# earth-system-radiation/rte-ecckd

Measured on AMD Instinct MI355X. Metric: Mcol*lay*gpt/s LW gas_optics+rte_lw, higher is better.
Workload: dtype f64

## Files before the change

rte-ecckd_amd/csrc/capi.cpp:

```cpp
#include <hip/hip_runtime.h>

#include <atomic>
#include <cmath>
#include <cstdint>
#include <cstdlib>
#include <cstring>
#include <map>
#include <mutex>
#include <string>
#include <vector>

#include "../../include/ecckd_hip.h"
#include "kernels.hpp"
#include "model.hpp"

namespace {

thread_local std::string g_err;

int fail(const std::string &msg) {
  g_err = msg;
  return 1;
}
}
// ... 205 lines not shown

struct Bump {
  char *base;
  size_t es;
  size_t off = 0;
  Bump(void *b, bool f32) : base(static_cast<char *>(b)), es(esz(f32)) {}
  double *take(size_t nelem) {
    double *r = reinterpret_cast<double *>(base + off);
    off += align256(nelem * es);
    return r;
  }
};

struct GasDesc {
  int ngas;
  const char *names;
  const double *const *vmr;
  const long long *cs, *ls;
  const double *scalar;
};

size_t vmr_extent(const GasDesc &gd, int j, int ncol, int nlay) {
  if (!gd.vmr || !gd.vmr[j]) return 0;
  const long long cs = gd.cs ? gd.cs[j] : 0, ls = gd.ls ? gd.ls[j] : 0;
  return (size_t)(1 + (long long)(ncol - 1) * cs + (long long)(nlay - 1) * ls);
}

struct PlanckSide {
  const double *tlev, *tsfc;
  double *lay_source, *lev_inc, *lev_dec, *sfc_source;
};

ecckd::PlanckArgs planck_args(const ecckd_model *m, int ncol, int nlay, const double *tlay, const PlanckSide &pl) {
  ecckd::PlanckArgs p{};
  p.ncol = ncol; p.nlay = nlay; p.ng = m->ng; p.ntp = m->ntp;
  p.planck = m->dbuf + m->off_planck;
  p.t0 = m->temperature_planck[0];
  p.dt = m->temperature_planck[1] - m->temperature_planck[0];
  p.tlay = tlay; p.tlev = pl.tlev; p.tsfc = pl.tsfc;
  p.lay_source = pl.lay_source; p.lev_source_inc = pl.lev_inc; p.lev_source_dec = pl.lev_dec;
  p.sfc_source = pl.sfc_source;
  return p;
}

int planck_sources_dev(const ecckd_model *m, int ncol, int nlay, const double *tlay, const PlanckSide &pl,
                       hipStream_t stream) {
  ecckd::PlanckArgs p = planck_args(m, ncol, nlay, tlay, pl);
  ProfScope prof("planck", stream);
  if (g_arith.load() == 0) HIPCHK(ecckd::launch_planck_pair(p, 0, stream));
  else HIPCHK(ecckd::launch_planck(p, stream));
  return 0;
}

int gas_optical_depth_dev(const ecckd_model *m, bool f32, PlanRecord *plan, int ncol, int nlay, const double *plev,
                          const double *tlay, const GasDesc &gd, double *tau, bool sw, double *ssa,
                          double *g, const PlanckSide *pl, bool *planck_done, hipStream_t stream) {
  using namespace ecckd;
  if (planck_done) *planck_done = false;
  std::vector<SeqGas> seq;
  bool first_calc = true;
  for (int j = 0; j < gd.ngas; ++j) {
    const std::string name = trim_name(gd.names + (size_t)j * ECCKD_NAME_LEN);
    size_t i = 0;
    for (; i < m->gas.size(); ++i)
      if (m->gas[i].name == name) break;
    if (i >= m->gas.size()) continue;
    const ecckd_model::Gas &t = m->gas[i];
    if (t.composite_only && !first_calc) continue;
    SeqGas e{};
    e.coef = table(m, t.dev_off, f32);
    e.vmr = gd.vmr ? gd.vmr[j] : nullptr;
    e.cs = gd.cs ? gd.cs[j] : 0;
    e.ls = gd.ls ? gd.ls[j] : 0;
    e.scalar = gd.scalar ? gd.scalar[j] : 0.;
    if (plan) {
      const bool sc = plan->is_scalar && plan->is_scalar[j];
      e.vmr = sc ? nullptr : reinterpret_cast<const double *>(sizeof(double));
      e.scalar = 1.;
    }
    e.ref = t.ref;
    e.code = t.code;
    e.nv = t.nv;
    e.clamp = t.has_negative ? 1 : 0;
    if (t.code == ECCKD_LOOK_UP_TABLE) {
      e.mf0 = t.mole_fraction[0];
      e.log_mf0 = std::log(t.mole_fraction[0]);
      e.d_log_vmr = std::log(t.mole_fraction[1] / t.mole_fraction[0]);
    }
    seq.push_back(e);
    if (t.composite_only) first_calc = false;
  }

  const bool fast = g_arith.load() == 0;
  size_t pos = 0;
  bool first_pass = true;
  do {
    FusedArgs fa{};
    TauArgs &a = fa.tau;
    a.ncol = ncol; a.nlay = nlay; a.ng = m->ng; a.np = m->np; a.nt = m->nt;
    a.plev = plev; a.tlay = tlay;
    a.temperature = table(m, m->off_temperature, f32);
    a.zero = table(m, m->off_zero, f32);
    a.lp0 = m->log_pressure[0];
    a.dlp = m->log_pressure[1] - m->log_pressure[0];
    a.dt = m->temperature[m->np] - m->temperature[0];
    a.gw = gw(f32);
    a.lut = -1;
    a.merge_slot = -1;
    a.nmerge = 0;
    a.nbil = 0;
    a.nseq = 0;
    while (pos < seq.size()) {
      SeqGas e = seq[pos];
      if (a.nseq >= kTauPassGases) break;
      if (e.code == ECCKD_LOOK_UP_TABLE) {
        if (a.lut >= 0) break;
        a.lut = a.nseq;
      } else {
        e.slot = a.nbil;
        a.bil_seq[a.nbil++] = a.nseq;
      }
      a.seq[a.nseq++] = e;
      ++pos;
    }
    a.accumulate = first_pass ? 0 : 1;
    a.tau = tau;
    const bool last = pos >= seq.size();
    if (sw && last) {
      a.rayleigh = table(m, m->off_rayleigh, f32);
      a.ssa = ssa;
      a.g = g;
    }
    if (fast) {
      fa.mode = (sw && last) ? 2 : 0;
      if (g_opt.gas_merge_scalars.load() && !f32) merge_scalar_gases(a, f32);
      const int nv_lut = a.lut >= 0 ? a.seq[a.lut].nv : 0;
      int pass_clamp = 0;
      for (int k = 0; k < a.nseq; ++k) pass_clamp |= a.seq[k].clamp;
      if (pl && first_pass && !sw &&
          fused_planck_rows(a.ng, a.np, a.nt, a.nbil, nv_lut, m->ntp, pass_clamp, f32) > 0) {
        fa.mode = 1;
        fa.ntp = m->ntp;
        fa.planck = table(m, m->off_planck, f32);
        fa.pt0 = m->temperature_planck[0];
        fa.pdt = m->temperature_planck[1] - m->temperature_planck[0];
        fa.tlev = pl->tlev; fa.tsfc = pl->tsfc;
        fa.lay_source = pl->lay_source; fa.lev_source_inc = pl->lev_inc;
        fa.lev_source_dec = pl->lev_dec; fa.sfc_source = pl->sfc_source;
        if (planck_done) *planck_done = true;
      }
      fa.f32 = f32;
      ScratchLease flag_lease;
      fa.slab32 = (!f32 && !plan && m->f32_exact && fa.mode == 1) ? g_opt.gas_slab_f32.load() : 0;
      if (fa.slab32 == 2) fa.choose_buf = static_cast<int *>(stream_scratch_optional(m->device, stream, 256, flag_lease, g_flag_pool));
      if (f32 && ((fa.mode != 1 && fa.mode != 2) || !last || !first_pass))
        return fail("ecckd: single precision is implemented for one-pass gas optics (fused longwave, shortwave); this "
                    "model / gas list needs the multi-pass or unfused path");
      if (plan) {
        FusedPlan fp;
        HIPCHK(prepare_gas_fused(fa, fp));
        if (plan->npass == 0) { plan->first_fused = 1; plan->planck_fused = fa.mode == 1; plan->first = fp; }
        ++plan->npass;
      } else {
        ProfScope prof(fa.mode == 1 ? (f32 ? "gas_lw_fused_f32" : "gas_lw_fused") : "tau", stream);
        HIPCHK(launch_gas_fused(fa, stream));
      }
    } else {
      if (f32) return fail("ecckd: single precision needs the fast arithmetic mode (ecckd_set_arithmetic(0))");
      if (plan) {
        ++plan->npass;
      } else {
        ProfScope prof("tau", stream);
        HIPCHK(launch_tau(a, stream));
      }
    }
    first_pass = false;
  } while (pos < seq.size());
  return 0;
}

int check_model(const ecckd_model *m) {
  if (!m) return fail("ecckd: null model");
  if (!m->finalized) return fail("ecckd: model is not finalized");
  if (m->device < 0) return fail("ecckd: host-only model (device -1): no GPU, no compute (there is no CPU fallback)");
  return 0;
}

int check_dims(int ncol, int nlay) {
  if (ncol < 0 || nlay < 1) return fail("ecckd: bad ncol/nlay");
  return 0;
}
int check_gas_optics_dims(int ncol, int nlay) {
  if (check_dims(ncol, nlay)) return 1;
  if (((size_t)ncol * (size_t)nlay + (size_t)ncol) * sizeof(double) >= (size_t)0xFFFFFFF0u)
    return fail("ecckd: ncol*(nlay+1) too large for one call (limit 2^29 elements): split the column range");
  return 0;
}

struct StagedGases {
  std::vector<const double *> ptr;
  GasDesc gd;
};
size_t staged_gas_bytes(const GasDesc &gd, int ncol, int nlay, bool f32) {
  size_t b = 0;
  for (int j = 0; j < gd.ngas; ++j) b += align256(vmr_extent(gd, j, ncol, nlay) * esz(f32));
  return b;
}
int stage_gases(const GasDesc &gd, int ncol, int nlay, Bump &bump, hipStream_t s, StagedGases &out) {
  out.ptr.assign(gd.ngas, nullptr);
  for (int j = 0; j < gd.ngas; ++j) {
    const size_t n = vmr_extent(gd, j, ncol, nlay);
    if (!n) continue;
    double *d = bump.take(n);
    HIPCHK(hipMemcpyAsync(d, gd.vmr[j], n * bump.es, hipMemcpyHostToDevice, s));
    out.ptr[j] = d;
  }
  out.gd = gd;
  out.gd.vmr = out.ptr.data();
  return 0;
}

int h2d(double *d, const double *h, size_t n, bool f32, hipStream_t s) {
  HIPCHK(hipMemcpyAsync(d, h, n * esz(f32), hipMemcpyHostToDevice, s));
  return 0;
}
int d2h(double *h, const double *d, size_t n, bool f32, hipStream_t s) {
  HIPCHK(hipMemcpyAsync(h, d, n * esz(f32), hipMemcpyDeviceToHost, s));
  return 0;
}

int grow_arena(ecckd_model *m, size_t need) {
  if (need <= m->arena_bytes) return 0;
  HIPCHK(hipStreamSynchronize(m->host_stream));
  if (m->arena) { HIPCHK(hipFree(m->arena)); m->arena = nullptr; m->arena_bytes = 0; }
  HIPCHK(hipMalloc(&m->arena, need));
  m->arena_bytes = need;
  return 0;
}

template <class T> void sum_planes_host(const T *planes, int nplanes, size_t n, T *out) {
  for (size_t i = 0; i < n; ++i) {
    T acc = 0;
    for (int b = 0; b < nplanes; ++b) acc += planes[(size_t)b * n + i];
    out[i] = acc;
  }
}

int sum_planes(const double *planes, int nplanes, size_t n, double *out, bool f32, int memspace, void *stream) {
  if (memspace == ECCKD_DEVICE) {
    HIPCHK(ecckd::launch_sum_planes(planes, nplanes, n, out, f32, static_cast<hipStream_t>(stream)));
    return 0;
  }
  if (f32)
    sum_planes_host(reinterpret_cast<const float *>(planes), nplanes, n, reinterpret_cast<float *>(out));
  else
    sum_planes_host(planes, nplanes, n, out);
  return 0;
}
template <class T> T *el(T *p, size_t n, bool f32) { return reinterpret_cast<T *>(reinterpret_cast<uintptr_t>(p) + n * esz(f32)); }

int fill_band_map(int ngpt, int nband, const int *band2gpt, unsigned char *gpt2band) {
  if (ngpt < 1 || ngpt > 256) return fail("ecckd: ngpt must be in 1..256");
  if (nband < 1 || nband > 255 || !band2gpt) return fail("ecckd: bad band description");
  std::memset(gpt2band, 0, 256);
  std::vector<int> seen(ngpt, 0);
  for (int b = 0; b < nband; ++b) {
    const int lo = band2gpt[2 * b], hi = band2gpt[2 * b + 1];
    if (lo < 1 || hi > ngpt || lo > hi) return fail("ecckd: band2gpt out of range");
    for (int gpt = lo; gpt <= hi; ++gpt) { gpt2band[gpt - 1] = (unsigned char)b; seen[gpt - 1] = 1; }
  }
  for (int i = 0; i < ngpt; ++i)
    if (!seen[i]) return fail("ecckd: band2gpt does not cover every g-point");
  return 0;
}

}

extern "C" {

const char *ecckd_last_error(void) { return g_err.c_str(); }

const char *ecckd_build_info(void) {
  return "rte-ecckd hot path for MI355X: hipcc --offload-arch=gfx950 -O3 -ffp-contract=off, fp64";
}


int ecckd_device_malloc(int device, size_t bytes, void **ptr) {
  if (!ptr) return fail("ecckd_device_malloc: null output");
  *ptr = nullptr;
  int ndev = 0;
  if (hipGetDeviceCount(&ndev) != hipSuccess || ndev < 1)
    return fail("ecckd: no HIP device available (this library has no CPU fallback)");
  if (device < 0 || device >= ndev) return fail("ecckd_device_malloc: bad device ordinal");
  HIPCHK(hipSetDevice(device));
  if (bytes == 0) return 0;
  HIPCHK(hipMalloc(ptr, bytes));
  return 0;
}

int ecckd_device_free(int device, void *ptr) {
  if (!ptr) return 0;
  HIPCHK(hipSetDevice(device));
  HIPCHK(hipFree(ptr));
  return 0;
}

int ecckd_device_memcpy(int device, void *dst, const void *src, size_t bytes, int to_device) {
// ... 1310 lines not shown
```

rte-ecckd_amd/csrc/kernels.hpp:

```cpp
#pragma once
#include <hip/hip_runtime.h>

namespace ecckd {

constexpr int kMaxSeq = 16;
constexpr int kTauPassGases = 10;
constexpr int kLdsBudget = 160 * 1024;

struct SeqGas {
  const double *coef;
  const double *vmr;
  long long cs, ls;
  double scalar;
  double ref;
  double mf0;
  double log_mf0;
  double d_log_vmr;
  int code;
  int nv;
  int slot;
  int clamp;
};

struct TauArgs {
  int ncol, nlay, ng, np, nt;
  const double *plev, *tlay;
  const double *temperature;
  const double *zero;
  double lp0, dlp, dt, gw;
  int nseq;
  SeqGas seq[kMaxSeq];
  int nbil;
  int bil_seq[kMaxSeq];
  int lut;
  int merge_slot;
  int nmerge;
  int merge_seq[kMaxSeq];
  double merge_mult[kMaxSeq];
  int accumulate;
  double *tau;
  const double *rayleigh;
  double *ssa, *g;
  int R;
  int col_chunks;
  int seg;
};

struct UDiv { double d, r; int exact; };

struct SlotArgs {
  const double *vmr;
  long long ls;
  unsigned cs_bytes;
  double alpha, beta;
};

struct FusedArgs {
  TauArgs tau;
  UDiv ud_dlp, ud_dt, ud_dlv, ud_pdt;
  SlotArgs slot[kTauPassGases + 1];
  int f32;
  int slab32;
  int *choose_buf;
  const int *choose;
  int choose_total;
  int mode;
  int ntp;
  int pw;
  const double *planck;
  double pt0, pdt;
  const double *tlev, *tsfc;
  double *lay_source, *lev_source_inc, *lev_source_dec, *sfc_source;
};

struct PlanckArgs {
  int ncol, nlay, ng, ntp;
  const double *planck;
  double t0, dt;
  const double *tlay, *tlev, *tsfc;
  double *lay_source, *lev_source_inc, *lev_source_dec, *sfc_source;
  int lev_chunks;
};

struct RteLwArgs {
  int ncol, nlay, ng, top_at_1, nmus;
  double Ds[4], wts[4];
  const double *tau, *lay_source, *lev_source_inc, *lev_source_dec, *sfc_source;
  const double *sfc_emis;
  int nband;
  unsigned char gpt2band[256];
  double *flux_up, *flux_dn;
  double *scratch;
  int f32;
  int shared_levels;
  const double *inc_flux;
  double tau_thresh;
  int series3;
  int inc_isotropic;
  int use_split;
  int split_seg;
  long tail_first = -1;
  double *partials = nullptr;
};

struct RteSwArgs {
  int ncol, nlay, ng, top_at_1;
  const double *tau, *ssa, *g, *mu0, *toa;
  const double *alb_dir, *alb_dif;
  int nband;
  unsigned char gpt2band[256];
  double *flux_up, *flux_dn, *flux_dir;
  double *scratch;
  int exact_division;
  double k_floor;
  int dir_clamp;
  long tail_first = -1;
  double *partials = nullptr;
  int f32 = 0;
  int use_sys = 0;
  long sys_tail_first = -1;
  int sys_gchunk = 0;
  int sys_npark = 0;
  unsigned sys_park_at = 0;
  int derive = 0;
  const double *plev = nullptr, *rayleigh = nullptr, *solar = nullptr;
  const double *toa_scale = nullptr;
  double gw = 0.;
};

struct RteGptArgs {
  int ncol, nlay, ng, top_at_1, nmus;
  double Ds[4], wts[4];
  const double *tau, *lay_source, *lev_source_inc, *lev_source_dec, *sfc_emis, *sfc_src, *inc_flux;
  const double *ssa, *g, *mu0, *fdir_top, *inc_dif, *alb_dir, *alb_dif;
  double *flux_up, *flux_dn, *flux_dir;
  double tau_thresh, k_floor;
  int series3, inc_isotropic, dir_clamp;
};
hipError_t launch_lw_gpt(const RteGptArgs &a, hipStream_t s);
hipError_t launch_sw_gpt(const RteGptArgs &a, hipStream_t s);

int tau_slab_rows(int ng, int np, int nt, int nbil, int nv_lut);
size_t tau_lds_bytes(int ng, int np, int nt, int nbil, int nv_lut, int R);
size_t rte_lw_scratch_bytes(int ncol, int nlay, int ng);
size_t rte_lw_tail_plan(const RteLwArgs &a, int slots, long *tail_first);
size_t rte_sw_scratch_bytes(int ncol, int nlay, int ng);
size_t rte_sw_tail_plan(const RteSwArgs &a, long *tail_first, size_t *partials_at);

hipError_t launch_tau(TauArgs &a, hipStream_t s);
struct FusedPlan {
  int empty = 0;
  size_t lds_bytes = 0;
  int anyclamp = 0, GC = 0, NB = 0;
  int merged = 0;
  int slab_rows = 0, planck_rows = 0, col_chunks = 0;
};
hipError_t prepare_gas_fused(FusedArgs &a, FusedPlan &plan);
int merge_scalar_gases(TauArgs &t, int f32);
int fused_slab_rows(int ng, int np, int nt, int nbil, int nv_lut, int pl_rows, int min_rows, int anyclamp, int f32, int block = 0);
int fused_planck_rows(int ng, int np, int nt, int nbil, int nv_lut, int ntp, int anyclamp, int f32);
hipError_t launch_gas_fused(FusedArgs &a, hipStream_t s);
hipError_t launch_planck(PlanckArgs &a, hipStream_t s);
hipError_t launch_planck_pair(const PlanckArgs &a, int f32, hipStream_t s);
size_t planck_pair_lds_bytes(int ng, int ntp, int f32);
UDiv make_udiv(double d, int f32);
hipError_t launch_toa_src(const double *solar, int ncol, int ng, double *toa_src, int f32, hipStream_t s);
hipError_t launch_sum_planes(const double *planes, int nplanes, size_t n, double *out, int f32, hipStream_t s);
hipError_t launch_rte_lw(const RteLwArgs &a, hipStream_t s);
bool rte_lw_split_applies(const RteLwArgs &a);
bool rte_lw_planck_fits(int ng, int ntp);
hipError_t launch_rte_lw_split(const RteLwArgs &a, hipStream_t s);
hipError_t launch_rte_lw_planck(const RteLwArgs &a, const double *planck, int ntp, double t0, double dt, const double *tlay,
                                const double *tlev, const double *tsfc, hipStream_t s);
hipError_t launch_rte_sw(const RteSwArgs &a, hipStream_t s);
bool rte_sw_sys_applies(const RteSwArgs &a);
size_t rte_sw_sys_plan(RteSwArgs &a, int cus);
hipError_t launch_rte_sw_sys(const RteSwArgs &a, int cus, hipStream_t s);
hipError_t launch_rte_sw_tail_reduce(const RteSwArgs &a, int nchunks, int cw, long tail_first, long ntail, hipStream_t s);

}
```

rte-ecckd_amd/csrc/kernels_gas_fused.hip:

```cpp
#include <cstdlib>
#include <type_traits>

#include "kernels.hpp"
#include "wave_pair.hpp"

namespace ecckd {
namespace {

#ifndef ECCKD_FUSED_BLOCK
#define ECCKD_FUSED_BLOCK 512
#endif
constexpr int kBlock = ECCKD_FUSED_BLOCK;
#ifndef ECCKD_FUSED_BLOCK_SW
#define ECCKD_FUSED_BLOCK_SW 768
#endif
constexpr int kBlockSw = ECCKD_FUSED_BLOCK_SW;
#ifndef ECCKD_FUSED_SEG
#define ECCKD_FUSED_SEG 8
#endif
#ifndef ECCKD_FUSED_SEG_MAX
#define ECCKD_FUSED_SEG_MAX 64
#endif
constexpr int kSeg = ECCKD_FUSED_SEG;
constexpr int kSegMax = ECCKD_FUSED_SEG_MAX;

template <int I, int N, class F>
__device__ __forceinline__ void static_for(F &&f) {
  if constexpr (I < N) {
    f(std::integral_constant<int, I>{});
    static_for<I + 1, N>(f);
  }
}

constexpr int seq_item(int pos, int NLI, int NBI, int NPI) {
  if (NPI == 0 || pos < NLI) return pos;
  int r = pos - NLI, b = 0, k = 0;
  for (int q = 0;; ++q) {
    const bool planck_next = k < NPI && b >= ((2 * k + 1) * NBI) / (2 * NPI);
    if (q == r) return planck_next ? NLI + NBI + k : NLI + b;
    if (planck_next) ++k; else ++b;
  }
}
constexpr int bil_slot(int b, int NP2) { return b / NP2; }
constexpr int bil_pair(int b, int NP2) { return b % NP2; }

template <typename real> __device__ __forceinline__ real selmin(real a, real b) { return a < b ? a : b; }
template <typename real> __device__ __forceinline__ real selmax(real a, real b) { return a > b ? a : b; }

struct FLayout {
  int tb, red, bil, SB, lut, SL, pl, SP, total;
};

__host__ __device__ inline FLayout f_layout(int ngp, int np, int nt, int nbil, int NB, int nv_lut, int R, int ntp, int wide = 1, int waves = kBlock / 64) {
  FLayout L;
  L.tb = 0;
  L.red = (np + 1) & ~1;
  L.bil = L.red + 4 * waves * wide;
  L.SB = nbil > 0 ? row_stride(nbil * ngp) : 2;
  L.lut = L.bil + R * nt * L.SB + NB * ngp;
  L.SL = nv_lut > 0 ? row_stride(ngp) : 2;
  L.pl = L.lut + (nv_lut > 0 ? R * nt * nv_lut * L.SL : 0) + ngp;
  L.SP = row_stride(ngp);
  L.total = L.pl + (ntp > 0 ? ntp * L.SP : 0);
  return L;
}

template <typename real> struct PPoint { int ip0; real pw0, pw1; };
template <typename real> __device__ __forceinline__ PPoint<real> pressure_point(real p0, real p1, real lp0, const UDivT<real> &dlp, int np) {
  const real log_pressure = log(real(0.5) * (p1 + p0));
  real pressure_index = udiv(log_pressure - lp0, dlp);
  pressure_index = real(1) + selmax(real(0), selmin(pressure_index, (real)np - real(1.0001)));
  PPoint<real> r;
  r.ip0 = (int)pressure_index;
  r.pw1 = pressure_index - r.ip0;
  r.pw0 = real(1) - r.pw1;
  return r;
}

enum { MODE_TAU = 0, MODE_LW = 1, MODE_SW = 2 };
constexpr int fused_block(int mode) { return mode == MODE_LW ? kBlock : kBlockSw; }

constexpr int kSpreadOneIn = 24;
template <typename real>
__global__ void __launch_bounds__(256) spread_probe_kernel(const real *plev, int ncol, int nlay, real lp0, UDiv dlp_h, int np, int *count) {
  const real *plev0 = plev + (long)ncol * (blockIdx.y ? nlay - 1 : 0), *plev1 = plev0 + ncol;
  const UDivT<real> dlp = make_udiv_t<real>(dlp_h);
  const long c = (long)blockIdx.x * 256 + threadIdx.x;
  int ip = -1;
  if (c < ncol) ip = pressure_point<real>(plev0[c], plev1[c], lp0, dlp, np).ip0;
  int lo = ip < 0 ? 0x7fffffff : ip, hi = ip;
#pragma unroll
  for (int o = 32; o > 0; o >>= 1) {
    lo = min(lo, __shfl_xor(lo, o));
    hi = max(hi, __shfl_xor(hi, o));
  }
  if ((threadIdx.x & 63) == 0 && hi - lo >= 2) atomicAdd(count, 1);
}

#ifndef ECCKD_F64_WAVES
#define ECCKD_F64_WAVES 2
#endif
#ifndef ECCKD_F32_WAVES
#define ECCKD_F32_WAVES 2
#endif
template <typename real, int GC, int NB, bool FULL, bool ANYCLAMP, int MODE, typename sreal = real, int BLOCK = kBlock>
__global__ void __launch_bounds__(BLOCK, (BLOCK > 512 ? 3 : sizeof(real) == 4 ? ECCKD_F32_WAVES : ECCKD_F64_WAVES)) gas_fused_kernel(const FusedArgs a) {
  constexpr int kBlock = BLOCK, kWaves = BLOCK / 64;
  extern __shared__ __attribute__((aligned(16))) unsigned char lds_raw[];
  sreal *lds = reinterpret_cast<sreal *>(lds_raw);
  typedef sreal double2_t __attribute__((ext_vector_type(2)));
  typedef __attribute__((address_space(3))) const volatile sreal lds_cvd;
  typedef __attribute__((address_space(3))) const volatile double2_t lds_cvd2;
  lds_cvd *lv = (lds_cvd *)lds;
  typedef __attribute__((address_space(3))) const volatile char lds_cvc;
  auto ld2b = [&](int bytes, int elem) -> double2_t { return *(lds_cvd2 *)((lds_cvc *)lv + bytes + elem * (int)sizeof(sreal)); };
  constexpr int WIDE = (int)(sizeof(real) / sizeof(sreal));
  if (a.choose) {
    const bool want32 = (long)a.choose[0] * kSpreadOneIn > (long)a.choose_total;
    if (want32 != (WIDE == 2)) return;
  }
  const int tid = threadIdx.x, lane = tid & 63, wave = tid >> 6;
  const int wcol = (tid & ~63) + wave_column(lane);
  const int j = blockIdx.y;
  const TauArgs &t = a.tau;
  const int ncol = t.ncol, nlay = t.nlay, ng = t.ng, np = t.np, nt = t.nt, R = t.R;
  const int nv_lut = t.lut >= 0 ? t.seq[t.lut].nv : 0;
  const int ntp = MODE == MODE_LW ? a.ntp : 0;
  const int PW = MODE == MODE_LW ? a.pw : 0;
  const int ngp = (ng + GC - 1) / GC * GC;
  const FLayout L = f_layout(ngp, np, nt, t.nbil, NB, nv_lut, R, PW, WIDE, kWaves);
  real *redd = reinterpret_cast<real *>(lds + L.red);
  auto P = [](const double *p) { return reinterpret_cast<const real *>(p); };
  auto Q = [](double *p) { return reinterpret_cast<real *>(p); };
  const UDivT<real> ud_dlp = make_udiv_t<real>(a.ud_dlp), ud_dt = make_udiv_t<real>(a.ud_dt);
  const UDivT<real> ud_dlv = make_udiv_t<real>(a.ud_dlv), ud_pdt = make_udiv_t<real>(a.ud_pdt);
  const real lp0 = (real)t.lp0, gw = (real)t.gw, pt0 = (real)a.pt0;

  for (int i = tid; i < L.total; i += kBlock) lds[i] = sreal(0);
  __syncthreads();
  for (int i = tid; i < np; i += kBlock) lds[L.tb + i] = (sreal)P(t.temperature)[i];
  int pw_lo = -1;
  typedef __attribute__((address_space(1))) const char gcchar_t;
  typedef __attribute__((address_space(1))) const real greal_t;
  gcchar_t *slot_base[NB + 1];
  unsigned slot_cs[NB + 1];
#pragma unroll
  for (int s = 0; s <= NB; ++s) {
    const SlotArgs &e = a.slot[s < NB ? s : kTauPassGases];
    slot_base[s] = (gcchar_t *)(P(e.vmr) + (long)j * e.ls);
    slot_cs[s] = e.cs_bytes;
  }

  const long ntiles = ((long)ncol + kBlock - 1) / kBlock;
  const long t_begin = ntiles * blockIdx.x / gridDim.x;
  const long t_end = ntiles * (blockIdx.x + 1) / gridDim.x;
  int slab_lo = -1;
  const real *plev0 = P(t.plev) + (long)ncol * j, *plev1 = P(t.plev) + (long)ncol * (j + 1);
  const real pi = (real)3.14159265359f, rpi = real(1) / pi;

  const int seg_len = t.seg;
  for (long seg = t_begin; seg < t_end; seg += seg_len) {
    const long seg_end = seg + seg_len < t_end ? seg + seg_len : t_end;
    const bool windowed = MODE == MODE_LW && PW < ntp;
    real smin = real(3.0e38), smax = -real(3.0e38), tmin = real(3.0e38), tmax = -real(3.0e38);
    for (long tile = seg; tile < seg_end; ++tile) {
      const long c = tile * kBlock + tid;
      if (c < ncol) {
        const real sp = plev1[c] + plev0[c];
        smin = selmin(smin, sp);
        smax = selmax(smax, sp);
        if (windowed) {
          const real tl = P(t.tlay)[c + (long)ncol * j];
          tmin = selmin(tmin, tl);
          tmax = selmax(tmax, tl);
          if (a.tlev) {
            const real ta = P(a.tlev)[c + (long)ncol * j], tb = P(a.tlev)[c + (long)ncol * (j + 1)];
            tmin = selmin(tmin, selmin(ta, tb));
            tmax = selmax(tmax, selmax(ta, tb));
          }
        }
      }
    }
#pragma unroll
    for (int o = 32; o > 0; o >>= 1) {
      smin = selmin(smin, __shfl_xor(smin, o));
      smax = selmax(smax, __shfl_xor(smax, o));
      if (windowed) {
        tmin = selmin(tmin, __shfl_xor(tmin, o));
        tmax = selmax(tmax, __shfl_xor(tmax, o));
      }
    }
    __syncthreads();
    if (lane == 0) { redd[4 * wave] = smin; redd[4 * wave + 1] = smax; redd[4 * wave + 2] = tmin; redd[4 * wave + 3] = tmax; }
    __syncthreads();
    smin = redd[0]; smax = redd[1]; tmin = redd[2]; tmax = redd[3];
#pragma unroll
    for (int w = 1; w < kWaves; ++w) {
      smin = selmin(smin, redd[4 * w]); smax = selmax(smax, redd[4 * w + 1]);
      tmin = selmin(tmin, redd[4 * w + 2]); tmax = selmax(tmax, redd[4 * w + 3]);
    }
    if (MODE == MODE_LW) {
      int want = pw_lo;
      if (!windowed) {
        want = 0;
      } else if (tmin <= tmax) {
        const int rlo = planck_point<real>(tmin, pt0, ud_pdt, ntp).row, rhi = planck_point<real>(tmax, pt0, ud_pdt, ntp).row + 1;
        if (pw_lo < 0 || rlo < pw_lo || rhi > pw_lo + PW - 1) {
          const int slack = PW - (rhi - rlo + 1);
          want = rlo - (slack > 0 ? slack / 2 : 0);
          want = want < 0 ? 0 : (want > ntp - PW ? ntp - PW : want);
        }
      } else if (pw_lo < 0) {
        want = 0;
      }
      if (want != pw_lo) {
        pw_lo = want;
        for (int q = tid; q < PW * ng; q += kBlock) {
          const int r = q / ng, g = q - r * ng;
          lds[L.pl + r * L.SP + g] = (sreal)P(a.planck)[(long)(pw_lo + r) * ng + g];
        }
      }
    }
    int ipmin = 1, ipmax = 0;
    if (smin <= smax) {
      ipmin = pressure_point<real>(real(0), smin, lp0, ud_dlp, np).ip0;
      ipmax = pressure_point<real>(real(0), smax, lp0, ud_dlp, np).ip0;
    }
    auto merged_coef = [&](long o) -> real {
      real v = (real)t.merge_mult[0] * P(t.seq[t.merge_seq[0]].coef)[o];
      for (int k = 1; k < t.nmerge; ++k) v = fma((real)t.merge_mult[k], P(t.seq[t.merge_seq[k]].coef)[o], v);
      return v;
    };
    auto stage_slab = [&](int lo) {
      slab_lo = lo;
      const int rows_b = R * nt;
      const int items_b = rows_b * t.nbil;
      for (int q = wave; q < items_b; q += kWaves) {
        const int s = q % t.nbil, rb = q / t.nbil;
        const int ipl = rb % R, it = rb / R;
        const long row = (long)ng * ((slab_lo + ipl) + (long)np * it);
        sreal *dst = lds + L.bil + rb * L.SB + s * GC;
        const int cs = t.nbil * GC;
        if (s == t.merge_slot) {
          for (int g = lane; g < ng; g += 64) dst[(g / GC) * cs + g % GC] = (sreal)merged_coef(row + g);
        } else {
          const real *src = P(t.seq[t.bil_seq[s]].coef) + row;
          for (int g = lane; g < ng; g += 64) dst[(g / GC) * cs + g % GC] = (sreal)src[g];
        }
      }
      if (t.lut >= 0) {
        const real *coef = P(t.seq[t.lut].coef);
        const int rows_l = rows_b * nv_lut;
        for (int q = wave; q < rows_l; q += kWaves) {
          const int ipl = q % R, itv = q / R;
          const real *src = coef + (long)ng * ((slab_lo + ipl) + (long)np * itv);
          sreal *dst = lds + L.lut + q * L.SL;
          for (int g = lane; g < ng; g += 64) dst[g] = (sreal)src[g];
        }
      }
    };
    const int span = R >= 2 ? R - 1 : 1;
    const int npos = (R >= 2 && ipmin <= ipmax) ? (ipmax - ipmin + span) / span : 1;
    for (int pos = 0; pos < npos; ++pos) {
    const int pos_lo = npos > 1 ? ipmin + pos * span : -0x40000000;
    const int pos_hi = npos > 1 ? pos_lo + span - 1 : 0x40000000;
    if (pos > 0) __syncthreads();
    if (R >= 2 && ipmin <= ipmax) {
      if (npos > 1) {
        const int lo = min(pos_lo - 1, np - R);
        if (lo != slab_lo) stage_slab(lo);
      } else if (!(slab_lo >= 0 && ipmin - 1 >= slab_lo && ipmax <= slab_lo + R - 1)) {
        stage_slab(min(ipmin - 1, np - R));
      }
    }
    __syncthreads();

    real nx_p0, nx_p1, nx_T, nx_W[NB], nx_vlut, nx_Tl0 = real(0), nx_Tl1 = real(0);
    auto load_inputs = [&](long tile) {
      const long c = tile * kBlock + wcol;
      const unsigned cc32 = (unsigned)(c < ncol ? c : (long)ncol - 1);
      const unsigned co = cc32 * (unsigned)sizeof(real);
      auto at = [&](const real *row) { return *reinterpret_cast<greal_t *>((gcchar_t *)row + co); };
      nx_p0 = at(plev0); nx_p1 = at(plev1);
      nx_T = at(P(t.tlay) + (long)ncol * j);
#pragma unroll
      for (int s = 0; s < NB; ++s) nx_W[s] = *reinterpret_cast<greal_t *>(slot_base[s] + cc32 * slot_cs[s]);
      nx_vlut = *reinterpret_cast<greal_t *>(slot_base[NB] + cc32 * slot_cs[NB]);
      if (MODE == MODE_LW && a.tlev) {
        nx_Tl0 = at(P(a.tlev) + (long)ncol * j);
        nx_Tl1 = at(P(a.tlev) + (long)ncol * (j + 1));
      }
    };

    for (long tile = seg; tile < seg_end; ++tile) {
      const long c = tile * kBlock + wcol;
      const bool valid = c < ncol;
      const bool upper = lane >= 32;
      const long cc = c < ncol ? c : (long)ncol - 1;
      load_inputs(tile);
      const real p0 = nx_p0, p1 = nx_p1, Tlayer = nx_T;
      real W[NB];
#pragma unroll
      for (int s = 0; s < NB; ++s) W[s] = nx_W[s];
      real vlut = nx_vlut;
      const real Tl0 = nx_Tl0, Tl1 = nx_Tl1;

      const PPoint<real> pp = pressure_point<real>(p0, p1, lp0, ud_dlp, np);
      const int ip0 = pp.ip0;
      const int ipq = ipmin <= ipmax ? (ip0 < ipmin ? ipmin : (ip0 > ipmax ? ipmax : ip0)) : ip0;
      const bool own = valid && ipq >= pos_lo && ipq <= pos_hi;
      if (!__any(own)) {
        continue;
      }
      const bool lowest = !__any(valid && ipq < pos_lo);
      const bool stray_wave = __any(valid && (ipq != ip0 || ipmin > ipmax));
      int ipl = ip0 - 1 - slab_lo;
      const bool inslab = (R >= 2) && slab_lo >= 0 && ipl >= 0 && ipl + 1 <= R - 1;
      ipl = ipl < 0 ? 0 : (ipl > R - 2 ? (R >= 2 ? R - 2 : 0) : ipl);

      const real t0 = pp.pw0 * (real)lds[L.tb + ip0 - 1] + pp.pw1 * (real)lds[L.tb + ip0];
      real temperature_index = udiv(Tlayer - t0, ud_dt);
      temperature_index = real(1) + selmax(real(0), selmin(temperature_index, (real)nt - real(1.0001)));
      const int it0 = (int)temperature_index;
      const real tw1 = temperature_index - it0;
      const real tw0 = real(1) - tw1;
      const real dp = p1 - p0;
      const real simple_weight = gw * dp;

      const real a00 = tw0 * pp.pw0, a10 = tw0 * pp.pw1, a01 = tw1 * pp.pw0, a11 = tw1 * pp.pw1;
      real l000 = real(0), l100 = real(0), l010 = real(0), l110 = real(0), l001 = real(0), l101 = real(0), l011 = real(0), l111 = real(0);
      int iv0 = 1;
      if (t.lut >= 0) {
        const SeqGas &e = t.seq[t.lut];
        vlut = fma((real)a.slot[kTauPassGases].alpha, vlut, (real)a.slot[kTauPassGases].beta);
        const real log_vmr = log(selmax(vlut, (real)e.mf0));
        real vmr_index = udiv(log_vmr - (real)e.log_mf0, ud_dlv);
        vmr_index = real(1) + selmax(real(0), selmin(vmr_index, (real)e.nv - real(1.001)));
        iv0 = (int)vmr_index;
        const real vw1 = vmr_index - iv0, vw0 = real(1) - vw1;
        real wl = simple_weight * vlut;
        if (!ANYCLAMP) wl = wl < real(0) ? real(0) : wl;
        const real u0 = ANYCLAMP ? vw0 : wl * vw0, u1 = ANYCLAMP ? vw1 : wl * vw1;
        l000 = u0 * a00; l100 = u0 * a10; l010 = u0 * a01; l110 = u0 * a11;
        l001 = u1 * a00; l101 = u1 * a10; l011 = u1 * a01; l111 = u1 * a11;
        if (ANYCLAMP) vlut = wl;
      }
#pragma unroll
// ... 118 lines not shown
#pragma unroll
                  for (int q = 0; q < 2; ++q) {
                    real v = lutp[q];
                    v = fma(l001, (real)b[0][q], v); v = fma(l101, (real)b[1][q], v); v = fma(l011, (real)b[2][q], v);
                    v = fma(l111, (real)b[3][q], v);
                    if (ANYCLAMP) { v = vlut * v; v = v < real(0) ? real(0) : v; }
                    acc[g0 + q] = acc[g0 + q] + v;
                    asm volatile("" : "+v"(acc[g0 + q]));
                  }
                }
              } else if constexpr (pi_ < NLI + NBI) {
                constexpr int s = bil_slot(pi_ - NLI, NP2), g0 = 2 * bil_pair(pi_ - NLI, NP2);
#pragma unroll
                for (int q = 0; q < 2; ++q) {
                  real v = a00 * (real)b[0][q];
                  v = fma(a10, (real)b[1][q], v); v = fma(a01, (real)b[2][q], v); v = fma(a11, (real)b[3][q], v);
                  if (ANYCLAMP) { v = W[s] * v; v = v < real(0) ? real(0) : v; acc[g0 + q] = acc[g0 + q] + v; }
                  else acc[g0 + q] = fma(W[s], v, acc[g0 + q]);
                  asm volatile("" : "+v"(acc[g0 + q]));
                }
                if (pi_ == NLI + NBI - 1) {
#pragma unroll
                  for (int g = 0; g < GC; g += 2) {
                    const int npl = FULL ? 2 : ng - (gb + g);
                    if (FULL || npl >= 1) {
                      if (MODE == MODE_SW) {
                        const real r0 = moles * P(t.rayleigh)[gb + g], r1 = moles * P(t.rayleigh)[gb + g + 1];
                        const real t0_ = acc[g] + r0, t1_ = acc[g + 1] + r1;
                        store_pair<real>(w_tau, plane2, voff, coff, t0_, t1_, masked, active, npl, upper);
                        if (t.ssa) {
                          store_pair<real>(w_ssa, plane2, voff, coff, r0 / t0_, r1 / t1_, masked, active, npl, upper);
                          store_pair<real>(w_g, plane2, voff, coff, real(0), real(0), masked, active, npl, upper);
                        }
                      } else {
                        store_pair<real>(w_tau, plane2, voff, coff, acc[g], acc[g + 1], masked, active, npl, upper);
                      }
                    }
                  }
                }
              } else {
                constexpr int k = pi_ - NLI - NBI;
                constexpr int g = 2 * (k < NP2 ? k : k - NP2);
                const int npl = FULL ? 2 : ng - (gb + g);
                if constexpr (k < NP2) {
                  real vl[2], v1[2];
#pragma unroll
                  for (int q = 0; q < 2; ++q) {
                    vl[q] = div_pi(qlay.w0 * (real)b[0][q] + qlay.w1 * (real)b[1][q], pi, rpi);
                    v1[q] = div_pi(ql1.w0 * (real)b[2][q] + ql1.w1 * (real)b[3][q], pi, rpi);
                  }
                  if (FULL || npl >= 1) {
                    store_pair<real>(w_lay, plane2, voff, coff, vl[0], vl[1], masked, active, npl, upper);
                    if (a.tlev) {
                      store_pair<real>(w_inc, plane2, voff, coff, v1[0], v1[1], masked, active, npl, upper);
                      if (has_next) store_pair<real>(w_decn, plane2, voff, coff, v1[0], v1[1], masked, active, npl, upper);
                    }
                  }
                } else {
                  real v0[2];
#pragma unroll
                  for (int q = 0; q < 2; ++q) v0[q] = div_pi(ql0.w0 * (real)b[0][q] + ql0.w1 * (real)b[1][q], pi, rpi);
                  if (a.tlev && (FULL || npl >= 1)) store_pair<real>(w_dec0, plane2, voff, coff, v0[0], v0[1], masked, active, npl, upper);
                }
              }
            }
          });
#pragma unroll
          for (int q = 0; q < 4; ++q) ab[q] += cstride;
#pragma unroll
          for (int q = 0; q < 8; ++q) al[q] += ES * GC;
#pragma unroll
          for (int q = 0; q < 6; ++q) ap[q] += ES * GC;
        }
        };
        if (j == 0) {
          if (masked_wave) chunks(std::true_type{}, std::true_type{}); else chunks(std::false_type{}, std::true_type{});
        } else {
          if (masked_wave) chunks(std::true_type{}, std::false_type{}); else chunks(std::false_type{}, std::false_type{});
        }
      } else if (lowest) {
        int ip0 = ip0_, it0 = it0_, iv0 = iv0_;
        asm volatile("" : "+v"(ip0), "+v"(it0), "+v"(iv0));
        for (int g = 0; g < ng; ++g) {
          const long o = cc + (long)ncol * (j + (long)nlay * g);
          real acc = t.accumulate ? P(t.tau)[o] : real(0);
          if (t.lut >= 0) {
            const SeqGas &e = t.seq[t.lut];
            const real *cp = P(e.coef) + (long)ng * ((ip0 - 1) + (long)np * ((it0 - 1) + (long)nt * (iv0 - 1))) + g;
            const long dP = ng, dT = (long)ng * np, dV = (long)ng * np * nt;
            real v = l000 * cp[0];
            v = fma(l100, cp[dP], v);
            v = fma(l010, cp[dT], v);
            v = fma(l110, cp[dT + dP], v);
            v = fma(l001, cp[dV], v);
            v = fma(l101, cp[dV + dP], v);
            v = fma(l011, cp[dV + dT], v);
            v = fma(l111, cp[dV + dT + dP], v);
            if (ANYCLAMP) { v = vlut * v; v = v < real(0) ? real(0) : v; }
            acc = acc + v;
          }
#pragma unroll
          for (int s = 0; s < NB; ++s) {
            if (s < t.nbil) {
              const long o00 = (long)ng * ((ip0 - 1) + (long)np * (it0 - 1)) + g;
              const long dP = ng, dT = (long)ng * np;
              real c00, c10, c01, c11;
              if (s == t.merge_slot) {
                c00 = merged_coef(o00); c10 = merged_coef(o00 + dP); c01 = merged_coef(o00 + dT); c11 = merged_coef(o00 + dT + dP);
              } else {
                const real *cp = P(t.seq[t.bil_seq[s]].coef) + o00;
                c00 = cp[0]; c10 = cp[dP]; c01 = cp[dT]; c11 = cp[dT + dP];
              }
              real v = a00 * c00;
              v = fma(a10, c10, v);
              v = fma(a01, c01, v);
              v = fma(a11, c11, v);
              if (ANYCLAMP) { v = W[s] * v; v = v < real(0) ? real(0) : v; acc = acc + v; }
              else acc = fma(W[s], v, acc);
            }
          }
          if (valid) {
            if (MODE == MODE_SW) {
              const real ray = moles * P(t.rayleigh)[g];
              const real tt = acc + ray;
              Q(t.tau)[o] = tt;
              if (t.ssa) { Q(t.ssa)[o] = ray / tt; Q(t.g)[o] = real(0); }
            } else {
              Q(t.tau)[o] = acc;
            }
            if (MODE == MODE_LW) {
              const real *pg = P(a.planck) + g;
              Q(a.lay_source)[o] = div_pi(qlay.w0 * pg[(long)qlay.row * ng] + qlay.w1 * pg[(long)(qlay.row + 1) * ng], pi, rpi);
              if (a.tlev) {
                const real v1 = div_pi(ql1.w0 * pg[(long)ql1.row * ng] + ql1.w1 * pg[(long)(ql1.row + 1) * ng], pi, rpi);
                Q(a.lev_source_inc)[o] = v1;
                if (j + 1 < nlay) Q(a.lev_source_dec)[o + ncol] = v1;
                if (j == 0)
                  Q(a.lev_source_dec)[o] = div_pi(ql0.w0 * pg[(long)ql0.row * ng] + ql0.w1 * pg[(long)(ql0.row + 1) * ng], pi, rpi);
              }
            }
          }
        }
      }

      if (MODE == MODE_LW && j == 0 && mine) {
        const PlPoint<real> qs = planck_point<real>(P(a.tsfc)[c], pt0, ud_pdt, ntp);
        const real *p0r = P(a.planck) + (long)qs.row * ng, *p1r = p0r + ng;
        for (int g = 0; g < ng; ++g)
          Q(a.sfc_source)[c + (long)ncol * g] = div_pi(qs.w0 * p0r[g] + qs.w1 * p1r[g], pi, rpi);
      }
    }
    }
  }
}

template <typename real, int GC, int NB, bool FULL, bool ANYCLAMP, int MODE, typename sreal = real>
hipError_t launch_one(const FusedArgs &a, size_t lds_bytes, hipStream_t s) {
  constexpr int kBlock = fused_block(MODE);
  auto k = gas_fused_kernel<real, GC, NB, FULL, ANYCLAMP, MODE, sreal, kBlock>;
  hipError_t e = hipFuncSetAttribute(reinterpret_cast<const void *>(k),
                                     hipFuncAttributeMaxDynamicSharedMemorySize, (int)lds_bytes);
  if (e != hipSuccess) return e;
  hipLaunchKernelGGL(k, dim3(a.tau.col_chunks, a.tau.nlay), dim3(kBlock), lds_bytes, s, a);
  return hipGetLastError();
}

int pick_nb(int nbil) {
  if (nbil <= 2) return 2;
  if (nbil <= 5) return 5;
  if (nbil <= 7) return 7;
  return kTauPassGases;
}

template <typename real, int MODE>
hipError_t launch_mode(const FusedArgs &a, size_t lds, int NBsel, bool anyclamp, hipStream_t s) {
  const int ng = a.tau.ng;
  if (anyclamp && ng % 4 == 0) return launch_one<real, 4, kTauPassGases, true, true, MODE>(a, lds, s);
  if (anyclamp) return launch_one<real, 4, kTauPassGases, false, true, MODE>(a, lds, s);
  if (NBsel == 2 && ng % 8 == 0) return launch_one<real, 8, 2, true, false, MODE>(a, lds, s);
  if (NBsel == 2 && ng % 4 == 0) return launch_one<real, 4, 2, true, false, MODE>(a, lds, s);
  if (NBsel == 2) return launch_one<real, 4, 2, false, false, MODE>(a, lds, s);
  if (NBsel == 7 && ng % 8 == 0) return launch_one<real, 8, 7, true, false, MODE>(a, lds, s);
  if (NBsel == 7 && ng % 4 == 0) return launch_one<real, 4, 7, true, false, MODE>(a, lds, s);
  if (NBsel == 5 && ng % 4 == 0) return launch_one<real, 4, 5, true, false, MODE>(a, lds, s);
  if (NBsel == 5) return launch_one<real, 4, 5, false, false, MODE>(a, lds, s);
  if (ng % 4 == 0) return launch_one<real, 4, kTauPassGases, true, false, MODE>(a, lds, s);
  return launch_one<real, 4, kTauPassGases, false, false, MODE>(a, lds, s);
}

bool slab32_applies(int mode, int ng, int nbil, bool anyclamp) {
  return mode == MODE_LW && !anyclamp && ng % 8 == 0 && pick_nb(nbil) == 7;
}

void pick_shape(int ng, int nbil, bool anyclamp, int *GC, int *NB) {
  const int nb = pick_nb(nbil);
  if (anyclamp) { *GC = 4; *NB = kTauPassGases; }
  else if (nb == 2) { *GC = ng % 8 == 0 ? 8 : 4; *NB = 2; }
  else if (nb == 7 && ng % 8 == 0) { *GC = 8; *NB = 7; }
  else if (nb == 7 && ng % 4 == 0) { *GC = 4; *NB = 7; }
  else if (nb == 5) { *GC = 4; *NB = 5; }
  else { *GC = 4; *NB = kTauPassGases; }
}

}

int fused_slab_rows(int ng, int np, int nt, int nbil, int nv_lut, int pl_rows, int min_rows, int anyclamp, int f32, int block) {
  if (block <= 0) block = kBlock;
  int GC, NB;
  pick_shape(ng, nbil, anyclamp != 0, &GC, &NB);
  const int ngp = (ng + GC - 1) / GC * GC;
  const size_t esz = f32 ? sizeof(float) : sizeof(double);
  int R = 0;
  for (int r = 2; r <= np; ++r) {
    if (esz * (size_t)f_layout(ngp, np, nt, nbil, NB, nv_lut, r, pl_rows, f32 == 2 ? 2 : 1, block / 64).total <= (size_t)kLdsBudget) R = r;
    else break;
  }
  return R >= min_rows ? R : 0;
}

int fused_planck_rows(int ng, int np, int nt, int nbil, int nv_lut, int ntp, int anyclamp, int f32) {
  if (ntp < 2) return 0;
  if (const char *e = getenv("ECCKD_PLANCK_WINDOW")) {
    const int w = atoi(e);
    if (w >= 2 && w < ntp && fused_slab_rows(ng, np, nt, nbil, nv_lut, w, 3, anyclamp, f32) > 0) return w;
  }
  if (fused_slab_rows(ng, np, nt, nbil, nv_lut, ntp, 3, anyclamp, f32) > 0) return ntp;
  for (int w : {128, 96, 64, 48, 32, 16})
    if (w < ntp && fused_slab_rows(ng, np, nt, nbil, nv_lut, w, 3, anyclamp, f32) > 0) return w;
  return 0;
}

UDiv make_udiv(double d, int f32) {
  UDiv u;
  if (f32) d = (double)(float)d;
  u.d = d;
  u.r = f32 ? (double)(1.f / (float)d) : 1. / d;
  unsigned long long bits;
  static_assert(sizeof(bits) == sizeof(d), "");
  __builtin_memcpy(&bits, &d, 8);
  bool all_ones = (bits & 0xFFFFFFFFFFFFFULL) == 0xFFFFFFFFFFFFFULL;
  if (f32) {
    const float df = (float)d;
    unsigned int b32;
    __builtin_memcpy(&b32, &df, 4);
    all_ones = (b32 & 0x7FFFFFu) == 0x7FFFFFu;
  }
  u.exact = (d == d) && d != 0. && (d - d == 0.) && !all_ones && (u.r - u.r == 0.) ? 1 : 0;
  return u;
}

int merge_scalar_gases(TauArgs &t, int f32) {
  t.merge_slot = -1;
  t.nmerge = 0;
  int cand[kMaxSeq], ncand = 0;
  double mult[kMaxSeq];
  for (int s = 0; s < t.nbil; ++s) {
    const SeqGas &e = t.seq[t.bil_seq[s]];
    if (e.clamp) continue;
    double m;
    if (e.code == 0) m = 1.;
    else if (e.vmr) continue;
    else if (e.code == 3) m = f32 ? (double)((float)e.scalar - (float)e.ref) : e.scalar - e.ref;
    else m = f32 ? (double)(float)e.scalar : e.scalar;
    if (!(m >= 0.) || !(m - m == 0.)) continue;
    cand[ncand] = t.bil_seq[s];
    mult[ncand++] = m;
  }
  if (ncand < 2) return 0;
  int keep[kMaxSeq], nkeep = 0;
  for (int s = 0; s < t.nbil; ++s) {
    bool merged = false;
    for (int k = 0; k < ncand; ++k) merged |= cand[k] == t.bil_seq[s];
    if (!merged) keep[nkeep++] = t.bil_seq[s];
  }
  for (int s = 0; s < nkeep; ++s) { t.bil_seq[s] = keep[s]; t.seq[keep[s]].slot = s; }
  t.merge_slot = nkeep;
  t.bil_seq[nkeep] = cand[0];
  t.nbil = nkeep + 1;
  t.nmerge = ncand;
  for (int k = 0; k < ncand; ++k) { t.merge_seq[k] = cand[k]; t.merge_mult[k] = mult[k]; t.seq[cand[k]].slot = nkeep; }
  return ncand;
}

hipError_t prepare_gas_fused(FusedArgs &a, FusedPlan &plan) {
  TauArgs &t = a.tau;
  plan = FusedPlan{};
  a.ud_dlp = make_udiv(t.dlp, a.f32);
  a.ud_dt = make_udiv(t.dt, a.f32);
  a.ud_dlv = make_udiv(t.lut >= 0 ? t.seq[t.lut].d_log_vmr : 1., a.f32);
  a.ud_pdt = make_udiv(a.mode == MODE_LW ? a.pdt : 1., a.f32);
  const size_t esz = a.f32 ? sizeof(float) : sizeof(double);
  auto sub = [&](double x, double y) { return a.f32 ? (double)((float)x - (float)y) : x - y; };
  for (int s = 0; s <= kTauPassGases; ++s) {
    const int k = s < kTauPassGases ? (s < t.nbil ? t.bil_seq[s] : -1) : t.lut;
    SlotArgs &o = a.slot[s];
    o = SlotArgs{t.zero, 0, 0u, 0., 0.};
    if (s < kTauPassGases && s == t.merge_slot) {
      o.beta = 1.;
    } else if (k >= 0) {
      const SeqGas &e = t.seq[k];
      const bool arr = e.vmr != nullptr;
      if (arr) {
        if (e.cs < 0 || (unsigned long long)e.cs * (unsigned long long)(t.ncol > 0 ? t.ncol : 1) * esz >= 0xFFFFFFF0ull)
          return hipErrorInvalidValue;
        o.vmr = e.vmr; o.ls = e.ls; o.cs_bytes = (unsigned)((unsigned long long)e.cs * esz);
      }
      switch (e.code) {
        case 0: o.alpha = 0.; o.beta = 1.; break;
        case 3: o.alpha = arr ? 1. : 0.; o.beta = arr ? -e.ref : sub(e.scalar, e.ref); break;
        default: o.alpha = arr ? 1. : 0.; o.beta = arr ? 0. : e.scalar; break;
      }
    }
  }
  if (t.ncol <= 0 || t.nlay <= 0) { plan.empty = 1; return hipSuccess; }
  if (t.nseq > kTauPassGases) return hipErrorInvalidValue;
  if (((size_t)t.ncol * (size_t)t.nlay + (size_t)t.ncol) * (a.f32 ? sizeof(float) : sizeof(double)) >= (size_t)0xFFFFFFF0u)
// ... 81 lines not shown
```

Measured before the change: 85300.

## Make fused longwave gas-optics kernel persistent with an atomic work queue

The fused gas-optics kernel now launches a 1D grid capped at the number of resident blocks (CUs times occupancy) in LW mode. Each block loops over (layer, column-chunk) work items and claims the next one from a global atomic counter, which is zeroed with a memset before launch. The aim is to cut block launch and LDS setup cost (temperature table load, Planck window reuse) and balance load across CUs. It costs an extra memset, an atomic per item and some extra LDS for the next-item slot. Blocks also now carry the Planck window state across layers, which may change how often the window is reloaded.

```diff
diff --git a/rte-ecckd_amd/csrc/capi.cpp b/rte-ecckd_amd/csrc/capi.cpp
--- a/rte-ecckd_amd/csrc/capi.cpp
+++ b/rte-ecckd_amd/csrc/capi.cpp
@@ -381,7 +381,11 @@
       fa.f32 = f32;
       ScratchLease flag_lease;
       fa.slab32 = (!f32 && !plan && m->f32_exact && fa.mode == 1) ? g_opt.gas_slab_f32.load() : 0;
-      if (fa.slab32 == 2) fa.choose_buf = static_cast<int *>(stream_scratch_optional(m->device, stream, 256, flag_lease, g_flag_pool));
+      if (!plan) {
+        int *flags = static_cast<int *>(stream_scratch_optional(m->device, stream, 256, flag_lease, g_flag_pool));
+        fa.queue = flags;
+        if (fa.slab32 == 2 && flags) fa.choose_buf = flags + 1;
+      }
       if (f32 && ((fa.mode != 1 && fa.mode != 2) || !last || !first_pass))
         return fail("ecckd: single precision is implemented for one-pass gas optics (fused longwave, shortwave); this "
                     "model / gas list needs the multi-pass or unfused path");
diff --git a/rte-ecckd_amd/csrc/kernels.hpp b/rte-ecckd_amd/csrc/kernels.hpp
--- a/rte-ecckd_amd/csrc/kernels.hpp
+++ b/rte-ecckd_amd/csrc/kernels.hpp
@@ -64,6 +64,7 @@
   int *choose_buf;
   const int *choose;
   int choose_total;
+  int *queue;
   int mode;
   int ntp;
   int pw;
diff --git a/rte-ecckd_amd/csrc/kernels_gas_fused.hip b/rte-ecckd_amd/csrc/kernels_gas_fused.hip
--- a/rte-ecckd_amd/csrc/kernels_gas_fused.hip
+++ b/rte-ecckd_amd/csrc/kernels_gas_fused.hip
@@ -1,3 +1,4 @@
+#include <atomic>
 #include <cstdlib>
 #include <type_traits>
 
@@ -55,7 +56,7 @@
   FLayout L;
   L.tb = 0;
   L.red = (np + 1) & ~1;
-  L.bil = L.red + 4 * waves * wide;
+  L.bil = L.red + 4 * (waves + 1) * wide;
   L.SB = nbil > 0 ? row_stride(nbil * ngp) : 2;
   L.lut = L.bil + R * nt * L.SB + NB * ngp;
   L.SL = nv_lut > 0 ? row_stride(ngp) : 2;
@@ -121,7 +122,6 @@
   }
   const int tid = threadIdx.x, lane = tid & 63, wave = tid >> 6;
   const int wcol = (tid & ~63) + wave_column(lane);
-  const int j = blockIdx.y;
   const TauArgs &t = a.tau;
   const int ncol = t.ncol, nlay = t.nlay, ng = t.ng, np = t.np, nt = t.nt, R = t.R;
   const int nv_lut = t.lut >= 0 ? t.seq[t.lut].nv : 0;
@@ -140,8 +140,19 @@
   __syncthreads();
   for (int i = tid; i < np; i += kBlock) lds[L.tb + i] = (sreal)P(t.temperature)[i];
   int pw_lo = -1;
+  int slab_lo = -1;
   typedef __attribute__((address_space(1))) const char gcchar_t;
   typedef __attribute__((address_space(1))) const real greal_t;
+  const real pi = (real)3.14159265359f, rpi = real(1) / pi;
+  const long ntiles = ((long)ncol + kBlock - 1) / kBlock;
+  const int chunks = t.col_chunks, nitems = chunks * nlay;
+  int *next_item = reinterpret_cast<int *>(redd + 4 * kWaves);
+
+  const bool persistent = MODE == MODE_LW && a.queue != nullptr;
+  for (int item = blockIdx.x; item < nitems;) {
+  int claimed = 0;
+  if (persistent && tid == 0) claimed = atomicAdd(a.queue, 1);
+  const int j = item / chunks, xc = item - j * chunks;
   gcchar_t *slot_base[NB + 1];
   unsigned slot_cs[NB + 1];
 #pragma unroll
@@ -151,12 +162,10 @@
     slot_cs[s] = e.cs_bytes;
   }
 
-  const long ntiles = ((long)ncol + kBlock - 1) / kBlock;
-  const long t_begin = ntiles * blockIdx.x / gridDim.x;
-  const long t_end = ntiles * (blockIdx.x + 1) / gridDim.x;
-  int slab_lo = -1;
+  const long t_begin = ntiles * xc / chunks;
+  const long t_end = ntiles * (xc + 1) / chunks;
   const real *plev0 = P(t.plev) + (long)ncol * j, *plev1 = P(t.plev) + (long)ncol * (j + 1);
-  const real pi = (real)3.14159265359f, rpi = real(1) / pi;
+  int item_after = nitems;
 
   const int seg_len = t.seg;
   for (long seg = t_begin; seg < t_end; seg += seg_len) {
@@ -192,7 +201,9 @@
     }
     __syncthreads();
     if (lane == 0) { redd[4 * wave] = smin; redd[4 * wave + 1] = smax; redd[4 * wave + 2] = tmin; redd[4 * wave + 3] = tmax; }
+    if (persistent && tid == 0 && seg == t_begin) *next_item = (int)gridDim.x + claimed;
     __syncthreads();
+    if (persistent && seg == t_begin) item_after = *next_item;
     smin = redd[0]; smax = redd[1]; tmin = redd[2]; tmax = redd[3];
 #pragma unroll
     for (int w = 1; w < kWaves; ++w) {
@@ -617,6 +628,18 @@
     }
     }
   }
+  item = persistent ? item_after : nitems;
+  }
+}
+
+int device_cus(int dev) {
+  static std::atomic<int> cached[64];
+  if (dev < 0 || dev >= 64) return 0;
+  int v = cached[dev].load();
+  if (v > 0) return v;
+  if (hipDeviceGetAttribute(&v, hipDeviceAttributeMultiprocessorCount, dev) != hipSuccess || v <= 0) return 0;
+  cached[dev].store(v);
+  return v;
 }
 
 template <typename real, int GC, int NB, bool FULL, bool ANYCLAMP, int MODE, typename sreal = real>
@@ -626,7 +649,18 @@
   hipError_t e = hipFuncSetAttribute(reinterpret_cast<const void *>(k),
                                      hipFuncAttributeMaxDynamicSharedMemorySize, (int)lds_bytes);
   if (e != hipSuccess) return e;
-  hipLaunchKernelGGL(k, dim3(a.tau.col_chunks, a.tau.nlay), dim3(kBlock), lds_bytes, s, a);
+  long grid = (long)a.tau.col_chunks * a.tau.nlay;
+  if (MODE == MODE_LW && a.queue) {
+    int dev = 0, per_cu = 0;
+    if ((e = hipGetDevice(&dev)) != hipSuccess) return e;
+    const int cus = device_cus(dev);
+    if (cus <= 0) return hipErrorInvalidDevice;
+    if ((e = hipOccupancyMaxActiveBlocksPerMultiprocessor(&per_cu, k, kBlock, lds_bytes)) != hipSuccess) return e;
+    const long resident = (long)cus * (per_cu > 1 ? per_cu : 1);
+    if (resident < grid) grid = resident;
+    if ((e = hipMemsetAsync(a.queue, 0, sizeof(int), s)) != hipSuccess) return e;
+  }
+  hipLaunchKernelGGL(k, dim3((unsigned)grid), dim3(kBlock), lds_bytes, s, a);
   return hipGetLastError();
 }
 
```

Result: no change. 86230, median of 6 (+1.1%).
